# AnyLoc/AnyLoc

Hardware: NVIDIA H100
Metric: images/sec end-to-end DINOv2-VLAD descriptors (higher is better)
Workload: dtype f32-equivalent (tensor-core fp16 3-term split, fp32 accumulate)

## Files before the change

### anyloc_b200/_lib.py

```python
import ctypes as C
import os

import torch

_HERE = os.path.dirname(os.path.abspath(__file__))
LIB_PATH = os.path.join(_HERE, "libanyloc_b200.so")

DIST = {"cosine": 0, "euclidean": 1}
METRIC = {"cosine": 0, "l2": 1}
FACET = {"query": 0, "key": 1, "value": 2, "token": 3}
FFN = {"mlp": 0, "swiglufused": 1}
EPI = {"bias": 0, "bias_split": 1, "gelu_split": 2, "swiglu_split": 3, "ls_resid": 4}
ENGINE = {"auto": 0, "simt": 1, "tc3": 2}
PAIR = {"tf32": 0, "f16": 1}
ACT_SCALE = 8.0


class AnylocError(RuntimeError):
    pass


class VitCfg(C.Structure):
    _fields_ = [(n, C.c_int) for n in ("embed_dim", "depth", "num_heads", "ffn_kind", "ffn_hidden", "patch",
                                       "pair_dtype")]


_BLOCK_FIELDS = ["ln1_w", "ln1_b", "qkv_w_hi", "qkv_w_lo", "qkv_b", "proj_w_hi", "proj_w_lo", "proj_b",
                 "ls1", "ln2_w", "ln2_b", "in_w_hi", "in_w_lo", "in_b", "out_w_hi", "out_w_lo", "out_b", "ls2"]


class VitBlock(C.Structure):
    _fields_ = [(n, C.c_void_p) for n in _BLOCK_FIELDS] + \
               [(n, C.c_float) for n in ("qkv_alpha", "proj_alpha", "in_alpha", "out_alpha")]


class VitWeightsStruct(C.Structure):
    _fields_ = [("patch_w_hi", C.c_void_p), ("patch_w_lo", C.c_void_p), ("patch_b", C.c_void_p),
                ("cls_token", C.c_void_p), ("blocks", C.POINTER(VitBlock)), ("patch_alpha", C.c_float)]


_SIGS = {
    "anyloc_last_error": (C.c_char_p, []),
    "anyloc_version": (C.c_int, []),
    "anyloc_launch_count": (C.c_longlong, []),
    "anyloc_profile_enable": (C.c_int, [C.c_int]),
    "anyloc_profile_read": (C.c_int, [C.POINTER(C.c_double), C.POINTER(C.c_longlong), C.POINTER(C.c_double)]),
    "anyloc_device_info": (C.c_int, [C.POINTER(C.c_int), C.POINTER(C.c_size_t)]),
    "anyloc_vlad_workspace_bytes": (C.c_size_t, [C.c_int] * 4),
    "anyloc_vlad_generate": (C.c_int, [C.c_void_p, C.c_void_p, C.c_void_p] + [C.c_int] * 7 +
                             [C.c_void_p, C.c_void_p, C.c_void_p, C.c_size_t, C.c_void_p]),
    "anyloc_vlad_prepared_bytes": (C.c_size_t, [C.c_int] * 2),
    "anyloc_vlad_prepare": (C.c_int, [C.c_void_p, C.c_int, C.c_int, C.c_int, C.c_void_p, C.c_size_t, C.c_void_p]),
    "anyloc_vlad_generate_prepared": (C.c_int, [C.c_void_p, C.c_void_p, C.c_void_p, C.c_void_p, C.c_size_t] +
                                      [C.c_int] * 7 + [C.c_void_p, C.c_void_p, C.c_void_p, C.c_size_t, C.c_void_p]),
    "anyloc_vlad_generate_soft": (C.c_int, [C.c_void_p, C.c_void_p, C.c_void_p] + [C.c_int] * 4 + [C.c_float] +
                                  [C.c_int] * 2 + [C.c_void_p, C.c_void_p, C.c_void_p, C.c_size_t, C.c_void_p]),
    "anyloc_preprocess_u8": (C.c_int, [C.c_void_p] + [C.c_int] * 7 + [C.POINTER(C.c_float)] * 2 +
                             [C.c_void_p, C.c_void_p]),
    "anyloc_preprocess_resize_u8": (C.c_int, [C.c_void_p] + [C.c_int] * 10 + [C.POINTER(C.c_float)] * 2 +
                                    [C.c_void_p, C.c_void_p]),
    "anyloc_pool": (C.c_int, [C.c_void_p, C.c_void_p] + [C.c_int] * 4 + [C.c_float, C.c_int, C.c_void_p, C.c_void_p]),
    "anyloc_vlad_residuals": (C.c_int, [C.c_void_p, C.c_void_p] + [C.c_int] * 4 + [C.c_void_p, C.c_void_p]),
    "anyloc_vlad_from_residuals_workspace_bytes": (C.c_size_t, [C.c_int] * 2),
    "anyloc_vlad_from_residuals": (C.c_int, [C.c_void_p, C.c_void_p, C.c_void_p] + [C.c_int] * 4 +
                                   [C.c_void_p, C.c_void_p, C.c_size_t, C.c_void_p]),
    "anyloc_vlad_assign": (C.c_int, [C.c_void_p, C.c_void_p] + [C.c_int] * 4 +
                           [C.c_void_p, C.c_void_p, C.c_size_t, C.c_void_p]),
    "anyloc_kmeans_workspace_bytes": (C.c_size_t, [C.c_int] * 3),
    "anyloc_kmeans_update": (C.c_int, [C.c_void_p, C.c_void_p, C.c_void_p] + [C.c_int] * 3 +
                             [C.c_void_p, C.c_void_p, C.c_void_p, C.c_size_t, C.c_void_p]),
    "anyloc_kmeans_partition": (C.c_int, [C.c_int64, C.c_int, C.POINTER(C.c_int), C.POINTER(C.c_int64)]),
    "anyloc_kmeans_round_workspace_bytes": (C.c_size_t, [C.c_int64, C.c_int, C.c_int]),
    "anyloc_kmeans_accumulate_round": (C.c_int, [C.c_void_p, C.c_void_p, C.c_int64, C.c_int64, C.c_int64, C.c_int,
                                                 C.c_int, C.c_int, C.c_void_p, C.c_size_t, C.c_void_p]),
    "anyloc_kmeans_finalize": (C.c_int, [C.c_void_p, C.c_int64, C.c_int, C.c_int, C.c_void_p, C.c_void_p, C.c_void_p,
                                         C.c_size_t, C.c_void_p]),
    "anyloc_topk_workspace_bytes": (C.c_size_t, [C.c_int] * 4),
    "anyloc_topk": (C.c_int, [C.c_void_p, C.c_void_p] + [C.c_int] * 6 +
                    [C.c_void_p, C.c_void_p, C.c_void_p, C.c_size_t, C.c_void_p]),
    "anyloc_index_bytes": (C.c_size_t, [C.c_int64, C.c_int, C.c_int]),
    "anyloc_index_init": (C.c_int, [C.c_void_p, C.c_size_t, C.c_int64, C.c_int, C.c_int, C.c_void_p]),
    "anyloc_index_copy": (C.c_int, [C.c_void_p, C.c_size_t, C.c_int64, C.c_void_p, C.c_size_t, C.c_int64, C.c_int64,
                                    C.c_int, C.c_int, C.c_void_p]),
    "anyloc_index_add": (C.c_int, [C.c_void_p, C.c_size_t, C.c_int64, C.c_int64, C.c_void_p, C.c_int, C.c_int, C.c_int,
                                   C.c_void_p]),
    "anyloc_index_search_workspace_bytes": (C.c_size_t, [C.c_int64, C.c_int, C.c_int, C.c_int]),
    "anyloc_index_search": (C.c_int, [C.c_void_p, C.c_size_t, C.c_int64, C.c_int64, C.c_void_p] + [C.c_int] * 5 +
                            [C.c_void_p, C.c_void_p, C.c_void_p, C.c_size_t, C.c_void_p]),
    "anyloc_allgather_desc": (C.c_int, [C.c_void_p, C.c_void_p, C.c_void_p, C.c_size_t, C.c_int, C.c_void_p]),
    "anyloc_vit_patch_k": (C.c_int, [C.c_int]),
    "anyloc_vit_workspace_bytes": (C.c_size_t, [C.POINTER(VitCfg), C.c_int, C.c_int, C.c_int]),
    "anyloc_vit_extract": (C.c_int, [C.POINTER(VitCfg), C.POINTER(VitWeightsStruct), C.c_void_p,
                                     C.c_int, C.c_int, C.c_int, C.c_void_p, C.c_int, C.c_int, C.c_int,
                                     C.c_int, C.c_void_p, C.c_void_p, C.c_size_t, C.c_int, C.c_void_p]),
    "anyloc_gemm_nt": (C.c_int, [C.c_void_p, C.c_void_p, C.c_int, C.c_void_p, C.c_void_p, C.c_int,
                                 C.c_int, C.c_int, C.c_int, C.c_int, C.c_float, C.c_int, C.c_void_p, C.c_void_p,
                                 C.c_void_p, C.c_void_p, C.c_void_p, C.c_int, C.c_int, C.c_int, C.c_void_p]),
    "anyloc_split_tf32": (C.c_int, [C.c_void_p, C.c_void_p, C.c_void_p, C.c_size_t, C.c_void_p]),
    "anyloc_split_f16": (C.c_int, [C.c_void_p, C.c_void_p, C.c_void_p, C.c_size_t, C.c_float, C.c_void_p]),
    "anyloc_layernorm_split": (C.c_int, [C.c_void_p, C.c_void_p, C.c_void_p, C.c_int, C.c_int, C.c_float,
                                         C.c_void_p, C.c_void_p, C.c_int, C.c_void_p]),
    "anyloc_attention": (C.c_int, [C.c_void_p, C.c_void_p, C.c_int, C.c_int, C.c_int, C.c_int, C.c_void_p,
                                   C.c_void_p, C.c_int, C.c_int, C.c_void_p]),
    "anyloc_l2_normalize_rows": (C.c_int, [C.c_void_p, C.c_int64, C.c_int, C.c_int64, C.c_void_p, C.c_void_p]),
}
EXPORTS = sorted(_SIGS)

_lib = None


def load():
    global _lib
    if _lib is None:
        if not os.path.isfile(LIB_PATH):
            raise AnylocError(
                f"{LIB_PATH} is missing -- build it with `python -m anyloc_b200.build` "
                "(anyloc_b200 has no CPU fallback)")
        lib = C.CDLL(LIB_PATH)
        for name, (res, args) in _SIGS.items():
            fn = getattr(lib, name)
            fn.restype, fn.argtypes = res, args
        _lib = lib
    return _lib


def last_error():
    return load().anyloc_last_error().decode()


def check(rc, what):
    if rc != 0:
        raise AnylocError(f"{what} failed (rc={rc}): {last_error()}")


def require_cuda(device=None):
    if not torch.cuda.is_available():
        raise AnylocError("anyloc_b200 needs a CUDA device (sm_90a); there is no CPU fallback")
    load()
    dev = torch.device("cuda" if device is None else device)
    if dev.type != "cuda":
        raise AnylocError(f"anyloc_b200 runs on CUDA devices only (got device={device!r}); no CPU fallback")
    if dev.index is None:
        dev = torch.device("cuda", torch.cuda.current_device())
    return dev


def stream_ptr():
    return C.c_void_p(torch.cuda.current_stream().cuda_stream)


def ptr(t):
    if t is None:
        return C.c_void_p(0)
    assert t.is_cuda and t.is_contiguous(), "device-contiguous tensor required"
    return C.c_void_p(t.data_ptr())


class _WorkspacePool:

    def __init__(self):
        self._bufs = {}

    def get(self, device, nbytes, tag="default"):
        key = (device.index, tag)
        buf = self._bufs.get(key)
        if buf is None or buf.numel() < nbytes:
            self._bufs.pop(key, None)
            buf = None
            buf = torch.empty(int(nbytes), dtype=torch.uint8, device=device)
            self._bufs[key] = buf
        return buf

    def clear(self):
        self._bufs.clear()


workspaces = _WorkspacePool()

PROF_CATEGORIES = ["gemm_tc", "gemm_simt", "attention", "layernorm", "vit_misc", "vlad", "topk"]


def profile_enable(on=True):
    check(load().anyloc_profile_enable(int(bool(on))), "profile_enable")


def profile_read():
    n = len(PROF_CATEGORIES)
    ms, groups, work = (C.c_double * n)(), (C.c_longlong * n)(), (C.c_double * n)()
    check(load().anyloc_profile_read(ms, groups, work), "profile_read")
    return {c: (ms[i], groups[i], work[i]) for i, c in enumerate(PROF_CATEGORIES)}


def launch_count():
    return int(load().anyloc_launch_count())
```

### anyloc_b200/csrc/gemm_tc.cu

```cuda
#include <cuda.h>
#include <stdlib.h>
#include "epilogue.cuh"
#include "tc_common.cuh"

namespace anyloc {

namespace tc {

constexpr int BM = 128, BN = 128;
constexpr int KSTEPS = 4;
constexpr int A_BYTES = BM * 128;
constexpr int B_BYTES = BN * 128;
constexpr int THREADS = 384;

template <bool LO> struct Cfg {
  static constexpr int STAGE_BYTES = (LO ? 2 : 1) * (A_BYTES + B_BYTES);
  static constexpr int B_OFF = (LO ? 2 : 1) * A_BYTES;
  static constexpr int STAGES = LO ? 3 : 6;
  static constexpr int SMEM_BYTES = STAGES * STAGE_BYTES + 1024  + 256 ;
};
constexpr int CHUNK_KB_TF32 = 2;
constexpr int CHUNK_KB_F16 = 8;
constexpr int CHUNK_KB_COARSE = 32;

__device__ __forceinline__ void tile_coords(int tile, int num_m, int num_n, int band_n, int& m_blk, int& n_blk) {
  const int per_band = num_m * band_n;
  const int band = tile / per_band, r = tile - band * per_band;
  const int w = min(band_n, num_n - band * band_n);
  m_blk = r / w;
  n_blk = band * band_n + (r - m_blk * w);
}

__device__ __forceinline__ void store_split2(const EpiParams& ep, size_t o, float a, float b) {
  if (ep.out_f16) {
    uint32_t h, l;
    split_f16x2(a * kActScale, b * kActScale, h, l);
    *reinterpret_cast<uint32_t*>(reinterpret_cast<__half*>(ep.out) + o) = h;
    *reinterpret_cast<uint32_t*>(reinterpret_cast<__half*>(ep.out_lo) + o) = l;
  } else {
    float2 h, l;
    split_tf32(a, h.x, l.x); split_tf32(b, h.y, l.y);
    *reinterpret_cast<float2*>(ep.out + o) = h;
    *reinterpret_cast<float2*>(ep.out_lo + o) = l;
  }
}

__device__ __forceinline__ void epi_pair(const EpiParams& ep, int m, int n, int N, float v0, float v1) {
  const int mode = ep.mode;
  if (mode < 0) return;
  if (mode == ANYLOC_EPI_SWIGLU_SPLIT) {
    epi_store_pair(ep, m, n, v0, v1);
    return;
  }
  if (n + 1 >= N || (ep.ldo & 1)) {
    epi_store1(ep, m, n, v0);
    if (n + 1 < N) epi_store1(ep, m, n + 1, v1);
    return;
  }
  const float al = ep.alpha;
  float2 b = make_float2(0.f, 0.f);
  if (ep.bias) b = __ldg(reinterpret_cast<const float2*>(ep.bias + n));
  const float x0 = v0 * al + b.x, x1 = v1 * al + b.y;
  const size_t o = (size_t)m * ep.ldo + n;
  if (mode == ANYLOC_EPI_BIAS) {
    *reinterpret_cast<float2*>(ep.out + o) = make_float2(x0, x1);
  } else if (mode == ANYLOC_EPI_LS_RESID) {
    const float2 g = __ldg(reinterpret_cast<const float2*>(ep.gamma + n));
    const float2 r = *reinterpret_cast<const float2*>(ep.resid + o);
    *reinterpret_cast<float2*>(ep.out + o) = make_float2(r.x + g.x * x0, r.y + g.y * x1);
  } else if (mode == ANYLOC_EPI_GELU_SPLIT) {
    store_split2(ep, o, gelu_erf(x0), gelu_erf(x1));
  } else {
    store_split2(ep, o, x0, x1);
  }
}

__device__ __forceinline__ void epilogue_subtile(const EpiParams& ep, int r0, int nq, int M, int N, const float* sum) {
  const int mode = ep.mode;
  if (mode < 0) return;
  const int n0 = nq & ~(BN - 1);
  const bool swiglu = mode == ANYLOC_EPI_SWIGLU_SPLIT, resid = mode == ANYLOC_EPI_LS_RESID;
  if (n0 + BN > N || (!swiglu && (ep.ldo & 1))) {
#pragma unroll
    for (int j = 0; j < 16; ++j) {
      const int n = nq + j * 8;
      if (n >= N) continue;
      if (r0 < M) epi_pair(ep, r0, n, N, sum[4 * j], sum[4 * j + 1]);
      if (r0 + 8 < M) epi_pair(ep, r0 + 8, n, N, sum[4 * j + 2], sum[4 * j + 3]);
    }
    return;
  }
  const bool row0 = r0 < M, row1 = r0 + 8 < M;
  const size_t o0 = (size_t)r0 * ep.ldo, o1 = (size_t)(r0 + 8) * ep.ldo;
  const float al = ep.alpha;
#pragma unroll
  for (int j0 = 0; j0 < 16; j0 += 2) {
    float2 b[2], g[2], ra[2], rb[2];
#pragma unroll
    for (int jj = 0; jj < 2; ++jj) {
      const int n = nq + (j0 + jj) * 8;
      b[jj] = ep.bias ? __ldg(reinterpret_cast<const float2*>(ep.bias + n)) : make_float2(0.f, 0.f);
      if (resid) {
        g[jj] = __ldg(reinterpret_cast<const float2*>(ep.gamma + n));
        if (row0) ra[jj] = *reinterpret_cast<const float2*>(ep.resid + o0 + n);
        if (row1) rb[jj] = *reinterpret_cast<const float2*>(ep.resid + o1 + n);
      }
    }
#pragma unroll
    for (int jj = 0; jj < 2; ++jj) {
      const int j = j0 + jj, n = nq + j * 8;
#pragma unroll
      for (int h = 0; h < 2; ++h) {
        if (!(h ? row1 : row0)) continue;
        const float v0 = sum[4 * j + 2 * h], v1 = sum[4 * j + 2 * h + 1];
        const size_t ro = h ? o1 : o0;
        if (swiglu) {
          const float x1 = v0 * al + b[jj].x, x2 = v1 * al + b[jj].y;
          epi_store_split(ep, ro + (n >> 1), silu(x1) * x2);
          continue;
        }
        const float x0 = v0 * al + b[jj].x, x1 = v1 * al + b[jj].y;
        const size_t o = ro + n;
        if (mode == ANYLOC_EPI_BIAS) {
          *reinterpret_cast<float2*>(ep.out + o) = make_float2(x0, x1);
        } else if (resid) {
          const float2 r = h ? rb[jj] : ra[jj];
          *reinterpret_cast<float2*>(ep.out + o) = make_float2(r.x + g[jj].x * x0, r.y + g[jj].y * x1);
        } else if (mode == ANYLOC_EPI_GELU_SPLIT) {
          store_split2(ep, o, gelu_erf(x0), gelu_erf(x1));
        } else {
          store_split2(ep, o, x0, x1);
        }
      }
    }
  }
}

template <bool F16, int LOM>
__global__ void __launch_bounds__(THREADS, 1)
gemm_tc3_kernel(const __grid_constant__ CUtensorMap tm_a_hi, const __grid_constant__ CUtensorMap tm_a_lo,
                const __grid_constant__ CUtensorMap tm_b_hi, const __grid_constant__ CUtensorMap tm_b_lo,
                int M, int N, int K, int band_n, int chunk_kb, EpiParams ep) {
  constexpr bool LO = LOM != 0, has_a_lo = (LOM & 1) != 0, has_b_lo = (LOM & 2) != 0;
  using C = Cfg<LO>;
  if (ep.gate != nullptr && *reinterpret_cast<const volatile int*>(ep.gate) == 0) return;
  extern __shared__ uint8_t smem_raw[];
  uint8_t* smem = reinterpret_cast<uint8_t*>((reinterpret_cast<uintptr_t>(smem_raw) + 1023) & ~(uintptr_t)1023);
  uint64_t* full_bar = reinterpret_cast<uint64_t*>(smem + C::STAGES * C::STAGE_BYTES);
  uint64_t* empty_bar = full_bar + C::STAGES;

  const int wg = threadIdx.x >> 7;
  const int num_m = (M + BM - 1) / BM, num_n = (N + BN - 1) / BN;
  const int num_tiles = num_m * num_n;
  constexpr int BKE = F16 ? 64 : 32;
  const int num_k = (K + BKE - 1) / BKE;

  if (threadIdx.x == 0) {
    asm volatile("prefetch.tensormap [%0];" ::"l"(&tm_a_hi) : "memory");
    asm volatile("prefetch.tensormap [%0];" ::"l"(&tm_b_hi) : "memory");
    for (int s = 0; s < C::STAGES; ++s) { mbar_init(smem_u32(full_bar + s), 1); mbar_init(smem_u32(empty_bar + s), 2); }
    asm volatile("fence.mbarrier_init.release.cluster;" ::: "memory");
  }
  __syncthreads();

  if (wg == 0) {
    if (threadIdx.x == 0) {
      const uint32_t tx_bytes = A_BYTES * (1 + ((LO && has_a_lo) ? 1 : 0)) + B_BYTES * (1 + ((LO && has_b_lo) ? 1 : 0));
      int stage = 0; uint32_t phase = 0;
      for (int tile = blockIdx.x; tile < num_tiles; tile += gridDim.x) {
        int mb, nb; tile_coords(tile, num_m, num_n, band_n, mb, nb);
        const int m0 = mb * BM, n0 = nb * BN;
        for (int kb = 0; kb < num_k; ++kb) {
          mbar_wait(smem_u32(empty_bar + stage), phase ^ 1);
          const uint32_t fb = smem_u32(full_bar + stage);
          mbar_expect_tx(fb, tx_bytes);
          const uint32_t sbase = smem_u32(smem + stage * C::STAGE_BYTES);
          tma_load_2d(sbase, &tm_a_hi, fb, kb * BKE, m0);
          if (LO && has_a_lo) tma_load_2d(sbase + A_BYTES, &tm_a_lo, fb, kb * BKE, m0);
          tma_load_2d(sbase + C::B_OFF, &tm_b_hi, fb, kb * BKE, n0);
          if (LO && has_b_lo) tma_load_2d(sbase + C::B_OFF + B_BYTES, &tm_b_lo, fb, kb * BKE, n0);
          if (++stage == C::STAGES) { stage = 0; phase ^= 1; }
        }
      }
    }
    return;
  }

  const int t = threadIdx.x & 127, warp = t >> 5, lane = t & 31;
  const uint32_t a_sub = (uint32_t)(wg - 1) * 64 * 128;
  int stage = 0; uint32_t phase = 0;
  for (int tile = blockIdx.x; tile < num_tiles; tile += gridDim.x) {
    int mb, nb; tile_coords(tile, num_m, num_n, band_n, mb, nb);
    const int m0 = mb * BM + (wg - 1) * 64, n0 = nb * BN;
    float sum[64], acc[64];
#pragma unroll
    for (int j = 0; j < 64; ++j) { sum[j] = 0.f; acc[j] = 0.f; }
    int prev_stage = -1;
    for (int kb0 = 0; kb0 < num_k; kb0 += chunk_kb) {
      const int kb1 = min(num_k, kb0 + chunk_kb);
      for (int kb = kb0; kb < kb1; ++kb) {
        mbar_wait(smem_u32(full_bar + stage), phase);
        const uint32_t sbase = smem_u32(smem + stage * C::STAGE_BYTES);
        const uint64_t a_hi = make_desc(sbase + a_sub), a_lo = make_desc(sbase + A_BYTES + a_sub);
        const uint64_t b_hi = make_desc(sbase + C::B_OFF), b_lo = make_desc(sbase + C::B_OFF + B_BYTES);
        wgmma_fence();
#pragma unroll
        for (int k = 0; k < KSTEPS; ++k) {
          const uint64_t adv = (uint64_t)((k * 32) >> 4);
          wgmma_m64n128<F16>(acc, a_hi + adv, b_hi + adv, (kb != kb0 || k != 0) ? 1u : 0u);
          if (has_a_lo) wgmma_m64n128<F16>(acc, a_lo + adv, b_hi + adv, 1u);
          if (has_b_lo) wgmma_m64n128<F16>(acc, a_hi + adv, b_lo + adv, 1u);
        }
        wgmma_commit();
        wgmma_wait<1>();
        if (prev_stage >= 0 && t == 0) mbar_arrive(smem_u32(empty_bar + prev_stage));
        prev_stage = stage;
        if (++stage == C::STAGES) { stage = 0; phase ^= 1; }
      }
      wgmma_wait<0>();
      fence_regs<64>(acc);
#pragma unroll
      for (int j = 0; j < 64; ++j) sum[j] += acc[j];
    }
    if (t == 0) mbar_arrive(smem_u32(empty_bar + prev_stage));
    epilogue_subtile(ep, m0 + warp * 16 + (lane >> 2), n0 + 2 * (lane & 3), M, N, sum);
  }
}

typedef CUresult (*EncodeTiledFn)(CUtensorMap*, CUtensorMapDataType, cuuint32_t, void*, const cuuint64_t*,
                                  const cuuint64_t*, const cuuint32_t*, const cuuint32_t*, CUtensorMapInterleave,
                                  CUtensorMapSwizzle, CUtensorMapL2promotion, CUtensorMapFloatOOBfill);

static EncodeTiledFn get_encode() {
  static EncodeTiledFn fn = nullptr;
  if (!fn) {
    void* p = nullptr;
    cudaDriverEntryPointQueryResult q;
    if (cudaGetDriverEntryPoint("cuTensorMapEncodeTiled", &p, cudaEnableDefault, &q) != cudaSuccess ||
        q != cudaDriverEntryPointSuccess)
      return nullptr;
    fn = (EncodeTiledFn)p;
  }
  return fn;
}

int make_map(CUtensorMap* map, const void* ptr, int rows, int K, int ld, int box_rows, bool f16) {
  EncodeTiledFn enc = get_encode();
  if (!enc) { set_error("gemm_tc: cuTensorMapEncodeTiled unavailable"); return ANYLOC_ERR_CUDA; }
  const int esz = f16 ? 2 : 4;
  cuuint64_t dims[2] = {(cuuint64_t)K, (cuuint64_t)rows};
  cuuint64_t strides[1] = {(cuuint64_t)ld * esz};
  cuuint32_t box[2] = {(cuuint32_t)(128 / esz), (cuuint32_t)box_rows};
  cuuint32_t estr[2] = {1, 1};
  CUresult r = enc(map, f16 ? CU_TENSOR_MAP_DATA_TYPE_FLOAT16 : CU_TENSOR_MAP_DATA_TYPE_FLOAT32, 2, (void*)ptr, dims,
                   strides, box, estr, CU_TENSOR_MAP_INTERLEAVE_NONE, CU_TENSOR_MAP_SWIZZLE_128B,
                   CU_TENSOR_MAP_L2_PROMOTION_L2_256B, CU_TENSOR_MAP_FLOAT_OOB_FILL_NONE);
  if (r != CUDA_SUCCESS) { set_error("gemm_tc: cuTensorMapEncodeTiled failed (%d) rows=%d K=%d ld=%d", (int)r, rows, K, ld); return ANYLOC_ERR_CUDA; }
  return ANYLOC_OK;
}

}

bool gemm_tc_supported(const void* a_hi, const void* a_lo, int lda, const void* b_hi, const void* b_lo, int ldb,
                       int M, int N, int K, const EpiParams& ep, bool f16) {
  auto al16 = [](const void* p) { return (reinterpret_cast<uintptr_t>(p) & 15) == 0; };
  const int q = f16 ? 8 : 4;
  if (M < 1 || N < 1 || K < q) return false;
  if ((K % q) || (lda % q) || (ldb % q)) return false;
  if (!al16(a_hi) || !al16(b_hi) || (a_lo && !al16(a_lo)) || (b_lo && !al16(b_lo))) return false;
  if (!al16(ep.out) || (ep.out_lo && !al16(ep.out_lo)) || (ep.resid && !al16(ep.resid))) return false;
  if (ep.bias && !al16(ep.bias)) return false;
  if (ep.gamma && !al16(ep.gamma)) return false;
  return true;
}

template <bool F16, int LOM>
static int launch_impl(const void* a_hi, const void* a_lo, int lda, const void* b_hi, const void* b_lo, int ldb, int M,
                       int N, int K, const EpiParams& ep, int band_n, int chunk, cudaStream_t st) {
  using namespace tc;
  constexpr bool LO = LOM != 0;
  CUtensorMap ma_hi, ma_lo, mb_hi, mb_lo;
  int rc;
  if ((rc = make_map(&ma_hi, a_hi, M, K, lda, BM, F16))) return rc;
  if ((rc = make_map(&ma_lo, a_lo ? a_lo : a_hi, M, K, lda, BM, F16))) return rc;
  if ((rc = make_map(&mb_hi, b_hi, N, K, ldb, BN, F16))) return rc;
  if ((rc = make_map(&mb_lo, b_lo ? b_lo : b_hi, N, K, ldb, BN, F16))) return rc;
  static unsigned long long attr_seen = 0;
  if (first_use_on_this_device(&attr_seen)) {
    ANYLOC_CHECK_CUDA(cudaFuncSetAttribute(gemm_tc3_kernel<F16, LOM>, cudaFuncAttributeMaxDynamicSharedMemorySize,
                                           Cfg<LO>::SMEM_BYTES));
  }
  const int tiles = cdiv(M, BM) * cdiv(N, BN);
  const int grid = std::min(tiles, device_sm_count());
  gemm_tc3_kernel<F16, LOM><<<grid, THREADS, Cfg<LO>::SMEM_BYTES, st>>>(
      ma_hi, ma_lo, mb_hi, mb_lo, M, N, K, std::min(band_n, cdiv(N, BN)), chunk, ep);
  ANYLOC_CHECK_LAUNCH();
  return ANYLOC_OK;
}

int gemm_tc_launch(const void* a_hi, const void* a_lo, int lda, const void* b_hi, const void* b_lo, int ldb, int M,
                   int N, int K, const EpiParams& ep_in, bool f16, cudaStream_t st) {
  static int band_n = -1;
  if (band_n < 0) { const char* e = getenv("ANYLOC_GEMM_BAND"); band_n = e ? atoi(e) : 16; if (band_n < 1) band_n = 1 << 20; }
  static int chunk_env = -1;
  if (chunk_env < 0) { const char* e = getenv("ANYLOC_GEMM_CHUNK"); chunk_env = e ? atoi(e) : 0; }
  static int skip_epi = -1;
  if (skip_epi < 0) { const char* e = getenv("ANYLOC_GEMM_DEBUG_SKIP_EPI"); skip_epi = e ? atoi(e) : 0; }
  EpiParams ep = ep_in;
  if (skip_epi && ((skip_epi >> ep_in.mode) & 1)) ep.mode = -1;
  const int lom = (a_lo ? 1 : 0) | (b_lo ? 2 : 0);
  const int chunk = lom == 0 ? (f16 ? tc::CHUNK_KB_COARSE : tc::CHUNK_KB_TF32)
                             : chunk_env > 0 ? chunk_env : (f16 ? tc::CHUNK_KB_F16 : tc::CHUNK_KB_TF32);
#define ANYLOC_GEMM_LAUNCH(F16_, LOM_) launch_impl<F16_, LOM_>(a_hi, a_lo, lda, b_hi, b_lo, ldb, M, N, K, ep, band_n, chunk, st)
  switch (lom + (f16 ? 4 : 0)) {
    case 0: return ANYLOC_GEMM_LAUNCH(false, 0);
    case 1: return ANYLOC_GEMM_LAUNCH(false, 1);
    case 2: return ANYLOC_GEMM_LAUNCH(false, 2);
    case 3: return ANYLOC_GEMM_LAUNCH(false, 3);
    case 4: return ANYLOC_GEMM_LAUNCH(true, 0);
    case 5: return ANYLOC_GEMM_LAUNCH(true, 1);
    case 6: return ANYLOC_GEMM_LAUNCH(true, 2);
    default: return ANYLOC_GEMM_LAUNCH(true, 3);
  }
#undef ANYLOC_GEMM_LAUNCH
}

}
```

### anyloc_b200/csrc/tc_common.cuh

```cuda
#pragma once
#include <cuda.h>
#include "common.cuh"

namespace anyloc {
namespace tc {

__device__ __forceinline__ uint32_t smem_u32(const void* p) { return (uint32_t)__cvta_generic_to_shared(p); }

__device__ __forceinline__ void mbar_init(uint32_t bar, uint32_t count) {
  asm volatile("mbarrier.init.shared::cta.b64 [%0], %1;" ::"r"(bar), "r"(count));
}
__device__ __forceinline__ void mbar_expect_tx(uint32_t bar, uint32_t bytes) {
  asm volatile("mbarrier.arrive.expect_tx.shared::cta.b64 _, [%0], %1;" ::"r"(bar), "r"(bytes) : "memory");
}
__device__ __forceinline__ void mbar_arrive(uint32_t bar) {
  asm volatile("mbarrier.arrive.shared::cta.b64 _, [%0];" ::"r"(bar) : "memory");
}
__device__ __forceinline__ void mbar_wait(uint32_t bar, uint32_t parity) {
  uint32_t done = 0;
  long long t0 = 0;
  for (uint32_t it = 0; !done; ++it) {
    asm volatile(
        "{\n\t.reg .pred p;\n\t"
        "mbarrier.try_wait.parity.shared::cta.b64 p, [%1], %2;\n\t"
        "selp.u32 %0, 1, 0, p;\n\t}"
        : "=r"(done) : "r"(bar), "r"(parity) : "memory");
    if (!done && (it & 0x3ff) == 0x3ff) {
      long long now = clock64();
      if (t0 == 0) t0 = now;
      else if (now - t0 > 8000000000LL) __trap();
    }
  }
}
__device__ __forceinline__ void tma_load_2d(uint32_t dst, const CUtensorMap* map, uint32_t bar, int c0, int c1) {
  asm volatile(
      "cp.async.bulk.tensor.2d.shared::cluster.global.mbarrier::complete_tx::bytes [%0], [%1, {%3, %4}], [%2];"
      ::"r"(dst), "l"(map), "r"(bar), "r"(c0), "r"(c1) : "memory");
}

__device__ __forceinline__ uint64_t make_desc(uint32_t saddr) {
  uint64_t d = 0;
  d |= (uint64_t)((saddr & 0x3FFFF) >> 4);
  d |= (uint64_t)1 << 16;
  d |= (uint64_t)(1024 >> 4) << 32;
  d |= (uint64_t)1 << 62;
  return d;
}

__device__ __forceinline__ void wgmma_fence() { asm volatile("wgmma.fence.sync.aligned;" ::: "memory"); }
__device__ __forceinline__ void wgmma_commit() { asm volatile("wgmma.commit_group.sync.aligned;" ::: "memory"); }
template <int N>
__device__ __forceinline__ void wgmma_wait() { asm volatile("wgmma.wait_group.sync.aligned %0;" ::"n"(N) : "memory"); }
template <int R>
__device__ __forceinline__ void fence_regs(float* d) {
#pragma unroll
  for (int i = 0; i < R; ++i) asm volatile("" : "+f"(d[i])::"memory");
}

template <bool F16>
__device__ __forceinline__ void wgmma_m64n128(float* d, uint64_t adesc, uint64_t bdesc, uint32_t scale_d) {
  if constexpr (F16)
    asm volatile(
        "{\n\t.reg .pred p;\n\tsetp.ne.b32 p, %66, 0;\n\t"
        "wgmma.mma_async.sync.aligned.m64n128k16.f32.f16.f16 "
        "{%0, %1, %2, %3, %4, %5, %6, %7, %8, %9, %10, %11, %12, %13, %14, %15, %16, %17, %18, %19, %20, %21, %22, "
        "%23, %24, %25, %26, %27, %28, %29, %30, %31, %32, %33, %34, %35, %36, %37, %38, %39, %40, %41, %42, %43, %44, "
        "%45, %46, %47, %48, %49, %50, %51, %52, %53, %54, %55, %56, %57, %58, %59, %60, %61, %62, %63}, "
        "%64, %65, p, 1, 1, 0, 0;\n\t}"
        : "+f"(d[0]), "+f"(d[1]), "+f"(d[2]), "+f"(d[3]), "+f"(d[4]), "+f"(d[5]), "+f"(d[6]), "+f"(d[7]),
          "+f"(d[8]), "+f"(d[9]), "+f"(d[10]), "+f"(d[11]), "+f"(d[12]), "+f"(d[13]), "+f"(d[14]), "+f"(d[15]),
          "+f"(d[16]), "+f"(d[17]), "+f"(d[18]), "+f"(d[19]), "+f"(d[20]), "+f"(d[21]), "+f"(d[22]), "+f"(d[23]),
          "+f"(d[24]), "+f"(d[25]), "+f"(d[26]), "+f"(d[27]), "+f"(d[28]), "+f"(d[29]), "+f"(d[30]), "+f"(d[31]),
          "+f"(d[32]), "+f"(d[33]), "+f"(d[34]), "+f"(d[35]), "+f"(d[36]), "+f"(d[37]), "+f"(d[38]), "+f"(d[39]),
          "+f"(d[40]), "+f"(d[41]), "+f"(d[42]), "+f"(d[43]), "+f"(d[44]), "+f"(d[45]), "+f"(d[46]), "+f"(d[47]),
          "+f"(d[48]), "+f"(d[49]), "+f"(d[50]), "+f"(d[51]), "+f"(d[52]), "+f"(d[53]), "+f"(d[54]), "+f"(d[55]),
          "+f"(d[56]), "+f"(d[57]), "+f"(d[58]), "+f"(d[59]), "+f"(d[60]), "+f"(d[61]), "+f"(d[62]), "+f"(d[63])
        : "l"(adesc), "l"(bdesc), "r"(scale_d));
  else
    asm volatile(
        "{\n\t.reg .pred p;\n\tsetp.ne.b32 p, %66, 0;\n\t"
        "wgmma.mma_async.sync.aligned.m64n128k8.f32.tf32.tf32 "
        "{%0, %1, %2, %3, %4, %5, %6, %7, %8, %9, %10, %11, %12, %13, %14, %15, %16, %17, %18, %19, %20, %21, %22, "
        "%23, %24, %25, %26, %27, %28, %29, %30, %31, %32, %33, %34, %35, %36, %37, %38, %39, %40, %41, %42, %43, %44, "
        "%45, %46, %47, %48, %49, %50, %51, %52, %53, %54, %55, %56, %57, %58, %59, %60, %61, %62, %63}, "
        "%64, %65, p, 1, 1;\n\t}"
        : "+f"(d[0]), "+f"(d[1]), "+f"(d[2]), "+f"(d[3]), "+f"(d[4]), "+f"(d[5]), "+f"(d[6]), "+f"(d[7]),
          "+f"(d[8]), "+f"(d[9]), "+f"(d[10]), "+f"(d[11]), "+f"(d[12]), "+f"(d[13]), "+f"(d[14]), "+f"(d[15]),
          "+f"(d[16]), "+f"(d[17]), "+f"(d[18]), "+f"(d[19]), "+f"(d[20]), "+f"(d[21]), "+f"(d[22]), "+f"(d[23]),
          "+f"(d[24]), "+f"(d[25]), "+f"(d[26]), "+f"(d[27]), "+f"(d[28]), "+f"(d[29]), "+f"(d[30]), "+f"(d[31]),
          "+f"(d[32]), "+f"(d[33]), "+f"(d[34]), "+f"(d[35]), "+f"(d[36]), "+f"(d[37]), "+f"(d[38]), "+f"(d[39]),
          "+f"(d[40]), "+f"(d[41]), "+f"(d[42]), "+f"(d[43]), "+f"(d[44]), "+f"(d[45]), "+f"(d[46]), "+f"(d[47]),
          "+f"(d[48]), "+f"(d[49]), "+f"(d[50]), "+f"(d[51]), "+f"(d[52]), "+f"(d[53]), "+f"(d[54]), "+f"(d[55]),
          "+f"(d[56]), "+f"(d[57]), "+f"(d[58]), "+f"(d[59]), "+f"(d[60]), "+f"(d[61]), "+f"(d[62]), "+f"(d[63])
        : "l"(adesc), "l"(bdesc), "r"(scale_d));
}

int make_map(CUtensorMap* map, const void* ptr, int rows, int K, int ld, int box_rows, bool f16);

}
}
```

### include/anyloc_b200.h

```cpp
#ifndef ANYLOC_B200_H
#define ANYLOC_B200_H

#include <stddef.h>
#include <stdint.h>

#ifdef __cplusplus
extern "C" {
#endif

#define ANYLOC_OK 0
#define ANYLOC_ERR_ARG (-1)
#define ANYLOC_ERR_CUDA (-2)
#define ANYLOC_ERR_WORKSPACE (-3)
#define ANYLOC_ERR_UNSUPPORTED (-4)

#define ANYLOC_DIST_COSINE 0
#define ANYLOC_DIST_EUCLIDEAN 1
#define ANYLOC_METRIC_IP 0
#define ANYLOC_METRIC_L2 1
#define ANYLOC_FACET_QUERY 0
#define ANYLOC_FACET_KEY 1
#define ANYLOC_FACET_VALUE 2
#define ANYLOC_FACET_TOKEN 3
#define ANYLOC_FFN_MLP 0
#define ANYLOC_FFN_SWIGLU 1

#define ANYLOC_EPI_BIAS 0
#define ANYLOC_EPI_BIAS_SPLIT 1
#define ANYLOC_EPI_GELU_SPLIT 2
#define ANYLOC_EPI_SWIGLU_SPLIT 3
#define ANYLOC_EPI_LS_RESID 4
#define ANYLOC_PAIR_TF32 0
#define ANYLOC_PAIR_F16 1
#define ANYLOC_GEMM_AUTO 0
#define ANYLOC_GEMM_SIMT 1
#define ANYLOC_GEMM_TC3 2

const char* anyloc_last_error(void);
int anyloc_version(void);
int anyloc_device_info(int* sm_count, size_t* smem_optin_bytes);

#define ANYLOC_PROF_CATEGORIES 7
long long anyloc_launch_count(void);
int anyloc_profile_enable(int on);
int anyloc_profile_read(double* ms, long long* groups, double* work);

size_t anyloc_vlad_workspace_bytes(int B, int N, int D, int K);
int anyloc_vlad_generate(const float* feats, const int32_t* n_valid, const float* centers,
                         int B, int N, int D, int K, int dist_mode, int norm_descs, int intra_norm,
                         float* vlad, int32_t* labels, void* ws, size_t ws_bytes, void* stream);
size_t anyloc_vlad_prepared_bytes(int D, int K);
int anyloc_vlad_prepare(const float* centers, int D, int K, int dist_mode, void* prepared, size_t prepared_bytes,
                        void* stream);
int anyloc_vlad_generate_prepared(const float* feats, const int32_t* n_valid, const float* centers, void* prepared,
                                  size_t prepared_bytes, int B, int N, int D, int K, int dist_mode, int norm_descs,
                                  int intra_norm, float* vlad, int32_t* labels, void* ws, size_t ws_bytes, void* stream);
int anyloc_vlad_generate_soft(const float* feats, const int32_t* n_valid, const float* centers,
                              int B, int N, int D, int K, float soft_temp, int norm_descs, int intra_norm,
                              float* vlad, float* assign, void* ws, size_t ws_bytes, void* stream);
int anyloc_vlad_residuals(const float* feats, const float* centers, int N, int D, int K, int norm_descs,
                          float* out, void* stream);
size_t anyloc_vlad_from_residuals_workspace_bytes(int D, int K);
int anyloc_vlad_from_residuals(const float* resid, const int32_t* labels, const float* assign, int N, int D, int K,
                               int intra_norm, float* vlad, void* ws, size_t ws_bytes, void* stream);
int anyloc_vlad_assign(const float* feats, const float* centers, int R, int D, int K, int dist_mode,
                       int32_t* labels, void* ws, size_t ws_bytes, void* stream);
size_t anyloc_kmeans_workspace_bytes(int R, int D, int K);
int anyloc_kmeans_update(const float* x, const int32_t* labels, const float* old_centers, int R, int D,
                         int K, float* new_centers, float* err_out, void* ws, size_t ws_bytes,
                         void* stream);
int anyloc_kmeans_partition(int64_t R, int D, int* chunks, int64_t* rows_per);
size_t anyloc_kmeans_round_workspace_bytes(int64_t R, int D, int K);
int anyloc_kmeans_accumulate_round(const float* x, const int32_t* labels, int64_t R, int64_t round_rows,
                                   int64_t piece_rows, int D, int K, int resume, void* ws, size_t ws_bytes,
                                   void* stream);
int anyloc_kmeans_finalize(const float* old_centers, int64_t R, int D, int K, float* new_centers, float* err_out,
                           void* ws, size_t ws_bytes, void* stream);

size_t anyloc_topk_workspace_bytes(int n_db, int n_q, int Dv, int k);
int anyloc_topk(const float* db, const float* qu, int n_db, int n_q, int Dv, int k, int metric,
                int normalize, float* dist, int64_t* idx, void* ws, size_t ws_bytes, void* stream);

size_t anyloc_index_bytes(int64_t capacity, int Dv, int normalize);
int anyloc_index_init(void* index, size_t index_bytes, int64_t capacity, int Dv, int normalize, void* stream);
int anyloc_index_copy(void* dst, size_t dst_bytes, int64_t dst_capacity, const void* src, size_t src_bytes,
                      int64_t src_capacity, int64_t n_rows, int Dv, int normalize, void* stream);
int anyloc_index_add(void* index, size_t index_bytes, int64_t capacity, int64_t row_offset, const float* rows,
                     int n_rows, int Dv, int normalize, void* stream);
size_t anyloc_index_search_workspace_bytes(int64_t n_db, int n_q, int Dv, int normalize);
int anyloc_index_search(const void* index, size_t index_bytes, int64_t capacity, int64_t n_db, const float* qu,
                        int n_q, int Dv, int k, int metric, int normalize, float* dist, int64_t* idx, void* ws,
                        size_t ws_bytes, void* stream);

int anyloc_allgather_desc(void* nccl_comm, const float* local, float* all, size_t n_loc, int Dv, void* stream);

typedef struct {
  int embed_dim;
  int depth;
  int num_heads;
  int ffn_kind;
  int ffn_hidden;
  int patch;
  int pair_dtype;
} AnylocVitCfg;

typedef struct {
  const float *ln1_w, *ln1_b;
  const void *qkv_w_hi, *qkv_w_lo; const float *qkv_b;
  const void *proj_w_hi, *proj_w_lo; const float *proj_b;
  const float *ls1;
  const float *ln2_w, *ln2_b;
  const void *in_w_hi, *in_w_lo; const float *in_b;
  const void *out_w_hi, *out_w_lo; const float *out_b;
  const float *ls2;
  float qkv_alpha, proj_alpha, in_alpha, out_alpha;
} AnylocVitBlock;

typedef struct {
  const void *patch_w_hi, *patch_w_lo;
  const float *patch_b;
  const float *cls_token;
  const AnylocVitBlock* blocks;
  float patch_alpha;
} AnylocVitWeights;

int anyloc_vit_patch_k(int patch);
size_t anyloc_vit_workspace_bytes(const AnylocVitCfg* cfg, int B, int H, int W);
int anyloc_vit_extract(const AnylocVitCfg* cfg, const AnylocVitWeights* w_host, const float* img,
                       int B, int H, int W, const float* pos_embed, int layer, int facet,
                       int use_cls, int norm_descs, float* out, void* ws, size_t ws_bytes,
                       int gemm_engine, void* stream);

int anyloc_gemm_nt(const void* a_hi, const void* a_lo, int lda, const void* b_hi, const void* b_lo,
                   int ldb, int M, int N, int K, int in_dtype, float alpha, int epilogue, const float* bias,
                   const float* gamma, const float* resid, void* out, void* out_lo, int ldo, int out_dtype,
                   int engine, void* stream);
int anyloc_split_tf32(const float* x, float* hi, float* lo, size_t n, void* stream);
int anyloc_split_f16(const float* x, void* hi, void* lo, size_t n, float scale, void* stream);
int anyloc_layernorm_split(const float* x, const float* w, const float* b, int M, int D, float eps,
                           void* y_hi, void* y_lo, int out_dtype, void* stream);
int anyloc_attention(const float* qkv_hi, const float* qkv_lo, int B, int T, int D, int heads,
                     void* o_hi, void* o_lo, int out_dtype, int engine, void* stream);
int anyloc_l2_normalize_rows(const float* x, int64_t rows, int D, int64_t ld_in, float* y, void* stream);

#define ANYLOC_POOL_AVG 0
#define ANYLOC_POOL_MAX 1
#define ANYLOC_POOL_GEM 2
int anyloc_pool(const float* feats, const int32_t* n_valid, int B, int N, int D, int mode, float gem_p,
                int gem_use_abs, float* out, void* stream);

int anyloc_preprocess_u8(const uint8_t* img, int B, int H, int W, int top, int left, int Hc, int Wc,
                         const float* mean3, const float* std3, float* out, void* stream);
int anyloc_preprocess_resize_u8(const uint8_t* img, int B, int H, int W, int Hr, int Wr, int interpolation, int top,
                                int left, int Hc, int Wc, const float* mean3, const float* std3, float* out,
                                void* stream);

#ifdef __cplusplus
}
#endif
#endif
```

Before: 149.6.

## Stage GEMM epilogue through swizzled shared memory and store via TMA

For the LO (3-term split) GEMM variant, the epilogue now writes results into double-buffered swizzled shared-memory staging tiles and issues TMA bulk tensor stores, instead of scattered per-thread float2 global stores. For the layer-scale residual epilogue it also prefetches the residual tile with TMA during the last K chunk. This aims for coalesced, asynchronous output writes that overlap with the next tile's work. It costs extra shared memory and adds named barriers, mbarrier phase tracking and more tensor-map encoding on the host per launch.

New measurement: 167.3, median of 6. +11.8%, better.

```diff
diff --git a/anyloc_b200/_lib.py b/anyloc_b200/_lib.py
--- a/anyloc_b200/_lib.py
+++ b/anyloc_b200/_lib.py
@@ -96,6 +96,7 @@
     "anyloc_gemm_nt": (C.c_int, [C.c_void_p, C.c_void_p, C.c_int, C.c_void_p, C.c_void_p, C.c_int,
                                  C.c_int, C.c_int, C.c_int, C.c_int, C.c_float, C.c_int, C.c_void_p, C.c_void_p,
                                  C.c_void_p, C.c_void_p, C.c_void_p, C.c_int, C.c_int, C.c_int, C.c_void_p]),
+    "anyloc_gemm_tc_last_staged": (C.c_int, []),
     "anyloc_split_tf32": (C.c_int, [C.c_void_p, C.c_void_p, C.c_void_p, C.c_size_t, C.c_void_p]),
     "anyloc_split_f16": (C.c_int, [C.c_void_p, C.c_void_p, C.c_void_p, C.c_size_t, C.c_float, C.c_void_p]),
     "anyloc_layernorm_split": (C.c_int, [C.c_void_p, C.c_void_p, C.c_void_p, C.c_int, C.c_int, C.c_float,
diff --git a/anyloc_b200/csrc/gemm_tc.cu b/anyloc_b200/csrc/gemm_tc.cu
--- a/anyloc_b200/csrc/gemm_tc.cu
+++ b/anyloc_b200/csrc/gemm_tc.cu
@@ -12,12 +12,17 @@
 constexpr int A_BYTES = BM * 128;
 constexpr int B_BYTES = BN * 128;
 constexpr int THREADS = 384;
+constexpr int STG_BYTES = 8192;
 
 template <bool LO> struct Cfg {
   static constexpr int STAGE_BYTES = (LO ? 2 : 1) * (A_BYTES + B_BYTES);
   static constexpr int B_OFF = (LO ? 2 : 1) * A_BYTES;
   static constexpr int STAGES = LO ? 3 : 6;
-  static constexpr int SMEM_BYTES = STAGES * STAGE_BYTES + 1024  + 256 ;
+  static constexpr int BAR_OFF = STAGES * STAGE_BYTES;
+  static constexpr int SMEM_BYTES = BAR_OFF + 256 + 1024 ;
+  static constexpr bool STAGED = LO;
+  static constexpr int STG_OFF = BAR_OFF + 1024;
+  static constexpr int SMEM_BYTES_STAGED = STG_OFF + 4 * STG_BYTES + 1024 ;
 };
 constexpr int CHUNK_KB_TF32 = 2;
 constexpr int CHUNK_KB_F16 = 8;
@@ -75,19 +80,23 @@
   }
 }
 
-__device__ __forceinline__ void epilogue_subtile(const EpiParams& ep, int r0, int nq, int M, int N, const float* sum) {
+__device__ __forceinline__ void epilogue_pairs(const EpiParams& ep, int r0, int nq, int M, int N, const float* sum) {
+#pragma unroll
+  for (int j = 0; j < 16; ++j) {
+    const int n = nq + j * 8;
+    if (n >= N) continue;
+    if (r0 < M) epi_pair(ep, r0, n, N, sum[4 * j], sum[4 * j + 1]);
+    if (r0 + 8 < M) epi_pair(ep, r0 + 8, n, N, sum[4 * j + 2], sum[4 * j + 3]);
+  }
+}
+
+__device__ __forceinline__ void epilogue_regs_batched(const EpiParams& ep, int r0, int nq, int M, int N, const float* sum) {
   const int mode = ep.mode;
   if (mode < 0) return;
   const int n0 = nq & ~(BN - 1);
   const bool swiglu = mode == ANYLOC_EPI_SWIGLU_SPLIT, resid = mode == ANYLOC_EPI_LS_RESID;
   if (n0 + BN > N || (!swiglu && (ep.ldo & 1))) {
-#pragma unroll
-    for (int j = 0; j < 16; ++j) {
-      const int n = nq + j * 8;
-      if (n >= N) continue;
-      if (r0 < M) epi_pair(ep, r0, n, N, sum[4 * j], sum[4 * j + 1]);
-      if (r0 + 8 < M) epi_pair(ep, r0 + 8, n, N, sum[4 * j + 2], sum[4 * j + 3]);
-    }
+    epilogue_pairs(ep, r0, nq, M, N, sum);
     return;
   }
   const bool row0 = r0 < M, row1 = r0 + 8 < M;
@@ -136,18 +145,137 @@
   }
 }
 
+enum StageKind { STG_F32 = 0, STG_F16_PAIR = 1, STG_TF32_PAIR = 2 };
+constexpr int STG_HALF = STG_BYTES / 2;
+constexpr int STG_ROWS = 64;
+
+template <int KIND>
+struct StageFmt {
+  static constexpr int ESZ = KIND == STG_F16_PAIR ? 2 : 4;
+  static constexpr int COLS = KIND == STG_TF32_PAIR ? 16 : 32;
+  static constexpr int ROW_BYTES = COLS * ESZ;
+  static constexpr uint32_t SWZ = ROW_BYTES == 128 ? 7 : 3;
+};
+
+template <int KIND>
+__device__ __forceinline__ uint32_t stg_off(int row, int b) {
+  const uint32_t o = (uint32_t)(row * StageFmt<KIND>::ROW_BYTES + b);
+  return o ^ (((o >> 7) & StageFmt<KIND>::SWZ) << 4);
+}
+
+__device__ __forceinline__ float2 ldg_col_pair(const float* p, int n, int N) {
+  if (n + 1 < N) return __ldg(reinterpret_cast<const float2*>(p + n));
+  return make_float2(n < N ? __ldg(p + n) : 0.f, 0.f);
+}
+
+__device__ __forceinline__ void resid_load(const CUtensorMap* tm, uint8_t* buf, uint64_t* bar, int oc, int m0) {
+  mbar_expect_tx(smem_u32(bar), STG_BYTES);
+  tma_load_2d(smem_u32(buf), tm, smem_u32(bar), oc, m0);
+}
+
+template <int KIND, bool SWIGLU, bool RESID>
+__device__ __forceinline__ void epilogue_staged(const EpiParams& ep, const CUtensorMap* tm_out, const CUtensorMap* tm_lo,
+                                                const CUtensorMap* tm_resid, uint8_t* stg, uint64_t* rbar,
+                                                uint32_t& rphase, uint32_t& cnt, int wg, int t, int m0, int n0, int N,
+                                                const float* sum) {
+  using F = StageFmt<KIND>;
+  constexpr int ACC = SWIGLU ? 2 * F::COLS : F::COLS;
+  constexpr int JS = ACC / 8;
+  const int lane = t & 31, q = lane & 3, row = (t >> 5) * 16 + (lane >> 2);
+  const int n_out = SWIGLU ? N >> 1 : N;
+  const int oc_base = SWIGLU ? n0 >> 1 : n0;
+  const bool gelu = ep.mode == ANYLOC_EPI_GELU_SPLIT;
+  const float al = ep.alpha;
+#pragma unroll
+  for (int s = 0; s < BN / ACC; ++s) {
+    const int oc0 = oc_base + s * F::COLS;
+    if (oc0 >= n_out) break;
+    const uint32_t b = cnt & 1;
+    uint8_t* buf = stg + b * STG_BYTES;
+    if (RESID) { mbar_wait(smem_u32(rbar + b), (rphase >> b) & 1); rphase ^= 1u << b; }
+#pragma unroll
+    for (int jj = 0; jj < JS; ++jj) {
+      const int j = s * JS + jj, n = n0 + j * 8 + 2 * q;
+      const float2 bb = ep.bias ? ldg_col_pair(ep.bias, n, N) : make_float2(0.f, 0.f);
+      float2 g;
+      if (RESID) g = ldg_col_pair(ep.gamma, n, N);
+#pragma unroll
+      for (int h = 0; h < 2; ++h) {
+        const int r = row + 8 * h;
+        const float x0 = sum[4 * j + 2 * h] * al + bb.x, x1 = sum[4 * j + 2 * h + 1] * al + bb.y;
+        if (SWIGLU) {
+          const float v = silu(x0) * x1;
+          const uint32_t o = stg_off<KIND>(r, (4 * jj + q) * F::ESZ);
+          if (KIND == STG_F16_PAIR) {
+            __half hi, lo;
+            split_f16(v * kActScale, hi, lo);
+            *reinterpret_cast<__half*>(buf + o) = hi;
+            *reinterpret_cast<__half*>(buf + STG_HALF + o) = lo;
+          } else {
+            float hi, lo;
+            split_tf32(v, hi, lo);
+            *reinterpret_cast<float*>(buf + o) = hi;
+            *reinterpret_cast<float*>(buf + STG_HALF + o) = lo;
+          }
+          continue;
+        }
+        const uint32_t o = stg_off<KIND>(r, (8 * jj + 2 * q) * F::ESZ);
+        if (KIND == STG_F32) {
+          float2* p = reinterpret_cast<float2*>(buf + o);
+          if (RESID) {
+            const float2 rr = *p;
+            *p = make_float2(rr.x + g.x * x0, rr.y + g.y * x1);
+          } else {
+            *p = make_float2(x0, x1);
+          }
+        } else {
+          const float y0 = gelu ? gelu_erf(x0) : x0, y1 = gelu ? gelu_erf(x1) : x1;
+          if (KIND == STG_F16_PAIR) {
+            uint32_t hi, lo;
+            split_f16x2(y0 * kActScale, y1 * kActScale, hi, lo);
+            *reinterpret_cast<uint32_t*>(buf + o) = hi;
+            *reinterpret_cast<uint32_t*>(buf + STG_HALF + o) = lo;
+          } else {
+            float2 hi, lo;
+            split_tf32(y0, hi.x, lo.x); split_tf32(y1, hi.y, lo.y);
+            *reinterpret_cast<float2*>(buf + o) = hi;
+            *reinterpret_cast<float2*>(buf + STG_HALF + o) = lo;
+          }
+        }
+      }
+    }
+    fence_proxy_async_smem();
+    if (t == 0) bulk_wait_read<0>();
+    if (wg == 1) named_bar_sync<1>(128);
+    else named_bar_sync<2>(128);
+    if (t == 0) {
+      tma_store_2d(tm_out, smem_u32(buf), oc0, m0);
+      if (KIND != STG_F32) tma_store_2d(tm_lo, smem_u32(buf + STG_HALF), oc0, m0);
+      bulk_commit();
+      if (RESID && s + 2 < BN / ACC && oc0 + 2 * F::COLS < n_out) {
+        bulk_wait_read<0>();
+        resid_load(tm_resid, buf, rbar + b, oc0 + 2 * F::COLS, m0);
+      }
+    }
+    ++cnt;
+  }
+}
+
 template <bool F16, int LOM>
 __global__ void __launch_bounds__(THREADS, 1)
 gemm_tc3_kernel(const __grid_constant__ CUtensorMap tm_a_hi, const __grid_constant__ CUtensorMap tm_a_lo,
                 const __grid_constant__ CUtensorMap tm_b_hi, const __grid_constant__ CUtensorMap tm_b_lo,
+                const __grid_constant__ CUtensorMap tm_out, const __grid_constant__ CUtensorMap tm_out_lo,
+                const __grid_constant__ CUtensorMap tm_resid, int staged,
                 int M, int N, int K, int band_n, int chunk_kb, EpiParams ep) {
   constexpr bool LO = LOM != 0, has_a_lo = (LOM & 1) != 0, has_b_lo = (LOM & 2) != 0;
   using C = Cfg<LO>;
   if (ep.gate != nullptr && *reinterpret_cast<const volatile int*>(ep.gate) == 0) return;
   extern __shared__ uint8_t smem_raw[];
   uint8_t* smem = reinterpret_cast<uint8_t*>((reinterpret_cast<uintptr_t>(smem_raw) + 1023) & ~(uintptr_t)1023);
-  uint64_t* full_bar = reinterpret_cast<uint64_t*>(smem + C::STAGES * C::STAGE_BYTES);
+  uint64_t* full_bar = reinterpret_cast<uint64_t*>(smem + C::BAR_OFF);
   uint64_t* empty_bar = full_bar + C::STAGES;
+  uint64_t* resid_bar = empty_bar + C::STAGES;
 
   const int wg = threadIdx.x >> 7;
   const int num_m = (M + BM - 1) / BM, num_n = (N + BN - 1) / BN;
@@ -159,6 +287,8 @@
     asm volatile("prefetch.tensormap [%0];" ::"l"(&tm_a_hi) : "memory");
     asm volatile("prefetch.tensormap [%0];" ::"l"(&tm_b_hi) : "memory");
     for (int s = 0; s < C::STAGES; ++s) { mbar_init(smem_u32(full_bar + s), 1); mbar_init(smem_u32(empty_bar + s), 2); }
+    if (C::STAGED)
+      for (int i = 0; i < 4; ++i) mbar_init(smem_u32(resid_bar + i), 1);
     asm volatile("fence.mbarrier_init.release.cluster;" ::: "memory");
   }
   __syncthreads();
@@ -188,6 +318,12 @@
 
   const int t = threadIdx.x & 127, warp = t >> 5, lane = t & 31;
   const uint32_t a_sub = (uint32_t)(wg - 1) * 64 * 128;
+  uint8_t* stg = smem + C::STG_OFF + (wg - 1) * 2 * STG_BYTES;
+  uint64_t* rbar = resid_bar + (wg - 1) * 2;
+  const int mode = ep.mode;
+  staged = C::STAGED && staged;
+  const bool resid_staged = staged && mode == ANYLOC_EPI_LS_RESID;
+  uint32_t stg_cnt = 0, rphase = 0;
   int stage = 0; uint32_t phase = 0;
   for (int tile = blockIdx.x; tile < num_tiles; tile += gridDim.x) {
     int mb, nb; tile_coords(tile, num_m, num_n, band_n, mb, nb);
@@ -198,6 +334,14 @@
     int prev_stage = -1;
     for (int kb0 = 0; kb0 < num_k; kb0 += chunk_kb) {
       const int kb1 = min(num_k, kb0 + chunk_kb);
+      if (resid_staged && kb1 == num_k && t == 0 && m0 < M) {
+        bulk_wait_read<0>();
+        for (int i = 0; i < 2; ++i) {
+          const uint32_t b = (stg_cnt + i) & 1;
+          const int oc = n0 + i * StageFmt<STG_F32>::COLS;
+          if (oc < N) resid_load(&tm_resid, stg + b * STG_BYTES, rbar + b, oc, m0);
+        }
+      }
       for (int kb = kb0; kb < kb1; ++kb) {
         mbar_wait(smem_u32(full_bar + stage), phase);
         const uint32_t sbase = smem_u32(smem + stage * C::STAGE_BYTES);
@@ -223,8 +367,30 @@
       for (int j = 0; j < 64; ++j) sum[j] += acc[j];
     }
     if (t == 0) mbar_arrive(smem_u32(empty_bar + prev_stage));
-    epilogue_subtile(ep, m0 + warp * 16 + (lane >> 2), n0 + 2 * (lane & 3), M, N, sum);
-  }
+    if (mode < 0 || m0 >= M) continue;
+    if constexpr (!C::STAGED) {
+      epilogue_regs_batched(ep, m0 + warp * 16 + (lane >> 2), n0 + 2 * (lane & 3), M, N, sum);
+      continue;
+    }
+    if (!staged) {
+      epilogue_pairs(ep, m0 + warp * 16 + (lane >> 2), n0 + 2 * (lane & 3), M, N, sum);
+      continue;
+    }
+#define ANYLOC_EPI_STAGED(KIND_, SWIGLU_, RESID_)                                                                   \
+  epilogue_staged<KIND_, SWIGLU_, RESID_>(ep, &tm_out, &tm_out_lo, &tm_resid, stg, rbar, rphase, stg_cnt, wg, t, m0, \
+                                          n0, N, sum)
+    if (mode == ANYLOC_EPI_BIAS) ANYLOC_EPI_STAGED(STG_F32, false, false);
+    else if (mode == ANYLOC_EPI_LS_RESID) ANYLOC_EPI_STAGED(STG_F32, false, true);
+    else if (mode == ANYLOC_EPI_SWIGLU_SPLIT) {
+      if (ep.out_f16) ANYLOC_EPI_STAGED(STG_F16_PAIR, true, false);
+      else ANYLOC_EPI_STAGED(STG_TF32_PAIR, true, false);
+    } else {
+      if (ep.out_f16) ANYLOC_EPI_STAGED(STG_F16_PAIR, false, false);
+      else ANYLOC_EPI_STAGED(STG_TF32_PAIR, false, false);
+    }
+#undef ANYLOC_EPI_STAGED
+  }
+  if (staged && t == 0) bulk_wait<0>();
 }
 
 typedef CUresult (*EncodeTiledFn)(CUtensorMap*, CUtensorMapDataType, cuuint32_t, void*, const cuuint64_t*,
@@ -259,6 +425,38 @@
   return ANYLOC_OK;
 }
 
+static int make_out_map(CUtensorMap* map, const void* ptr, int rows, int cols, int ld, int esz, int box_cols) {
+  EncodeTiledFn enc = get_encode();
+  if (!enc) { set_error("gemm_tc: cuTensorMapEncodeTiled unavailable"); return ANYLOC_ERR_CUDA; }
+  cuuint64_t dims[2] = {(cuuint64_t)cols, (cuuint64_t)rows};
+  cuuint64_t strides[1] = {(cuuint64_t)ld * esz};
+  cuuint32_t box[2] = {(cuuint32_t)box_cols, (cuuint32_t)STG_ROWS};
+  cuuint32_t estr[2] = {1, 1};
+  CUresult r = enc(map, esz == 2 ? CU_TENSOR_MAP_DATA_TYPE_FLOAT16 : CU_TENSOR_MAP_DATA_TYPE_FLOAT32, 2, (void*)ptr,
+                   dims, strides, box, estr, CU_TENSOR_MAP_INTERLEAVE_NONE,
+                   box_cols * esz == 128 ? CU_TENSOR_MAP_SWIZZLE_128B : CU_TENSOR_MAP_SWIZZLE_64B,
+                   CU_TENSOR_MAP_L2_PROMOTION_L2_256B, CU_TENSOR_MAP_FLOAT_OOB_FILL_NONE);
+  if (r != CUDA_SUCCESS) { set_error("gemm_tc: cuTensorMapEncodeTiled failed (%d) for the output: rows=%d cols=%d ld=%d", (int)r, rows, cols, ld); return ANYLOC_ERR_CUDA; }
+  return ANYLOC_OK;
+}
+
+static int make_epi_maps(const EpiParams& ep, int M, int N, CUtensorMap* m_out, CUtensorMap* m_lo, CUtensorMap* m_resid,
+                         bool* staged) {
+  memset(m_out, 0, sizeof(*m_out)); memset(m_lo, 0, sizeof(*m_lo)); memset(m_resid, 0, sizeof(*m_resid));
+  const bool split = ep.mode == ANYLOC_EPI_BIAS_SPLIT || ep.mode == ANYLOC_EPI_GELU_SPLIT ||
+                     ep.mode == ANYLOC_EPI_SWIGLU_SPLIT;
+  const int esz = split && ep.out_f16 ? 2 : 4;
+  const int n_out = ep.mode == ANYLOC_EPI_SWIGLU_SPLIT ? N / 2 : N;
+  *staged = ep.mode >= 0 && ((long long)ep.ldo * esz) % 16 == 0 && ((long long)n_out * esz) % 16 == 0;
+  if (!*staged) return ANYLOC_OK;
+  const int cols = split && !ep.out_f16 ? StageFmt<STG_TF32_PAIR>::COLS : StageFmt<STG_F32>::COLS;
+  int rc;
+  if ((rc = make_out_map(m_out, ep.out, M, n_out, ep.ldo, esz, cols))) return rc;
+  if (split && (rc = make_out_map(m_lo, ep.out_lo, M, n_out, ep.ldo, esz, cols))) return rc;
+  if (ep.mode == ANYLOC_EPI_LS_RESID && (rc = make_out_map(m_resid, ep.resid, M, n_out, ep.ldo, esz, cols))) return rc;
+  return ANYLOC_OK;
+}
+
 }
 
 bool gemm_tc_supported(const void* a_hi, const void* a_lo, int lda, const void* b_hi, const void* b_lo, int ldb,
@@ -274,6 +472,8 @@
   return true;
 }
 
+static thread_local int g_last_staged = -1;
+
 template <bool F16, int LOM>
 static int launch_impl(const void* a_hi, const void* a_lo, int lda, const void* b_hi, const void* b_lo, int ldb, int M,
                        int N, int K, const EpiParams& ep, int band_n, int chunk, cudaStream_t st) {
@@ -285,15 +485,21 @@
   if ((rc = make_map(&ma_lo, a_lo ? a_lo : a_hi, M, K, lda, BM, F16))) return rc;
   if ((rc = make_map(&mb_hi, b_hi, N, K, ldb, BN, F16))) return rc;
   if ((rc = make_map(&mb_lo, b_lo ? b_lo : b_hi, N, K, ldb, BN, F16))) return rc;
+  CUtensorMap mo, mo_lo, mr;
+  bool staged = false;
+  memset(&mo, 0, sizeof(mo)); memset(&mo_lo, 0, sizeof(mo_lo)); memset(&mr, 0, sizeof(mr));
+  if (Cfg<LO>::STAGED && ep.gate == nullptr && (rc = make_epi_maps(ep, M, N, &mo, &mo_lo, &mr, &staged))) return rc;
+  const int smem = staged ? Cfg<LO>::SMEM_BYTES_STAGED : Cfg<LO>::SMEM_BYTES;
+  g_last_staged = staged ? 1 : 0;
   static unsigned long long attr_seen = 0;
   if (first_use_on_this_device(&attr_seen)) {
     ANYLOC_CHECK_CUDA(cudaFuncSetAttribute(gemm_tc3_kernel<F16, LOM>, cudaFuncAttributeMaxDynamicSharedMemorySize,
-                                           Cfg<LO>::SMEM_BYTES));
+                                           Cfg<LO>::STAGED ? Cfg<LO>::SMEM_BYTES_STAGED : Cfg<LO>::SMEM_BYTES));
   }
   const int tiles = cdiv(M, BM) * cdiv(N, BN);
   const int grid = std::min(tiles, device_sm_count());
-  gemm_tc3_kernel<F16, LOM><<<grid, THREADS, Cfg<LO>::SMEM_BYTES, st>>>(
-      ma_hi, ma_lo, mb_hi, mb_lo, M, N, K, std::min(band_n, cdiv(N, BN)), chunk, ep);
+  gemm_tc3_kernel<F16, LOM><<<grid, THREADS, smem, st>>>(
+      ma_hi, ma_lo, mb_hi, mb_lo, mo, mo_lo, mr, staged ? 1 : 0, M, N, K, std::min(band_n, cdiv(N, BN)), chunk, ep);
   ANYLOC_CHECK_LAUNCH();
   return ANYLOC_OK;
 }
@@ -326,3 +532,5 @@
 }
 
 }
+
+extern "C" int anyloc_gemm_tc_last_staged(void) { return anyloc::g_last_staged; }
diff --git a/anyloc_b200/csrc/tc_common.cuh b/anyloc_b200/csrc/tc_common.cuh
--- a/anyloc_b200/csrc/tc_common.cuh
+++ b/anyloc_b200/csrc/tc_common.cuh
@@ -36,6 +36,21 @@
   asm volatile(
       "cp.async.bulk.tensor.2d.shared::cluster.global.mbarrier::complete_tx::bytes [%0], [%1, {%3, %4}], [%2];"
       ::"r"(dst), "l"(map), "r"(bar), "r"(c0), "r"(c1) : "memory");
+}
+
+__device__ __forceinline__ void tma_store_2d(const CUtensorMap* map, uint32_t src, int c0, int c1) {
+  asm volatile("cp.async.bulk.tensor.2d.global.shared::cta.bulk_group [%0, {%2, %3}], [%1];"
+               ::"l"(map), "r"(src), "r"(c0), "r"(c1) : "memory");
+}
+__device__ __forceinline__ void bulk_commit() { asm volatile("cp.async.bulk.commit_group;" ::: "memory"); }
+template <int N>
+__device__ __forceinline__ void bulk_wait_read() { asm volatile("cp.async.bulk.wait_group.read %0;" ::"n"(N) : "memory"); }
+template <int N>
+__device__ __forceinline__ void bulk_wait() { asm volatile("cp.async.bulk.wait_group %0;" ::"n"(N) : "memory"); }
+__device__ __forceinline__ void fence_proxy_async_smem() { asm volatile("fence.proxy.async.shared::cta;" ::: "memory"); }
+template <int ID>
+__device__ __forceinline__ void named_bar_sync(int count) {
+  asm volatile("bar.sync %0, %1;" ::"n"(ID), "r"(count) : "memory");
 }
 
 __device__ __forceinline__ uint64_t make_desc(uint32_t saddr) {
diff --git a/include/anyloc_b200.h b/include/anyloc_b200.h
--- a/include/anyloc_b200.h
+++ b/include/anyloc_b200.h
@@ -135,6 +135,7 @@
                    int ldb, int M, int N, int K, int in_dtype, float alpha, int epilogue, const float* bias,
                    const float* gamma, const float* resid, void* out, void* out_lo, int ldo, int out_dtype,
                    int engine, void* stream);
+int anyloc_gemm_tc_last_staged(void);
 int anyloc_split_tf32(const float* x, float* hi, float* lo, size_t n, void* stream);
 int anyloc_split_f16(const float* x, void* hi, void* lo, size_t n, float scale, void* stream);
 int anyloc_layernorm_split(const float* x, const float* w, const float* b, int M, int D, float eps,
```
